# jdfxzzy/DPMN

Measured on AMD Instinct MI355X. Metric: SR images/sec (16x64->32x128, bs=48 per GPU, fp32 forward), higher is better.
Workload: dtype f32; 1 GPU; cfg1: TATT PSN + 3+3 PGRM (embed 96, windows 2/4/8) + CMM, forward-only; per_gpu_batch=48, global_batch=48, ranks=1, batches_in_flight=2, parallelism=dp1 (independent batch shards, no forward collective)

## Files before the change

dpmn_amd/_abi.py:

```python
import ctypes as C
import os

import torch

_HERE = os.path.dirname(os.path.abspath(__file__))
LIB_PATH = os.environ.get("DPMN_HIP_LIB") or os.path.join(_HERE, "lib", "libdpmn_hip.so")

if not os.path.exists(LIB_PATH):
    raise RuntimeError(
        "dpmn_amd: %s not found -- build it with `python -c 'import __graft_entry__ as g; g.build()'` "
        "(or `make -C dpmn_amd/csrc`).  There is no CPU fallback for the DPMN hot path." % LIB_PATH)

lib = C.CDLL(LIB_PATH)

fp = C.c_void_p


class PgrmBlock(C.Structure):
    _fields_ = [(n, fp) for n in (
        "norm1_q_w", "norm1_q_b", "norm1_kv_w", "norm1_kv_b", "q_w", "q_b", "kv_w", "kv_b")] + [
        ("bias_table", fp * 4)] + [(n, fp) for n in (
            "sk_proj_w", "sk_proj_b", "sk_fc1_w", "sk_fc1_b", "sk_fc2_w", "sk_fc2_b", "sk_head_w", "sk_head_b",
            "norm2_w", "norm2_b", "fc1_w", "fc1_b", "dw_w", "dw_b", "pw_w", "pw_b", "fc2_w", "fc2_b")]

# ... 114 lines not shown
    "dpmn_sk_mlp_in_supported": (_i, [_i, _i, _i, _i, _i]),
    "dpmn_pointwise_f32": (_i, [fp, fp, fp, fp, _i, _i, _i, fp]),
    "dpmn_conv2d_nhwc_f32": (_i, [C.POINTER(ConvDesc), fp]),
    "dpmn_distill_workspace_bytes": (_sz, [_i, _i, _i]),
    "dpmn_distill_forward_f32": (_i, [C.POINTER(DistillParams), fp, fp, _i, fp, fp, fp, fp, fp, _sz, _i, _i, _i, fp]),
    "dpmn_distill_backward_f32": (_i, [C.POINTER(DistillParams), C.POINTER(DistillGrads), fp, fp, fp, fp, fp, fp, fp, fp, fp, _sz, _i, _i, _i, fp]),
    "dpmn_conv2d_wgrad_unpack_multi_f32": (_i, [fp, fp, _i, _i, fp]),
    "dpmn_tl_interp_f32": (_i, [fp, fp, _i, _i, _i, _i, _i, fp]),
    "dpmn_pointwise_wgrad_det_bytes": (_sz, [_i, _i]),
    "dpmn_reduce_defer_begin": (_i, []),
    "dpmn_reduce_defer_enable": (_i, [_i]),
    "dpmn_reduce_defer_push": (_i, [C.POINTER(TnPending)]),
    "dpmn_reduce_defer_pending": (_i, []),
    "dpmn_reduce_defer_flush": (_i, [_i, fp]),
    "dpmn_xred_fallbacks": (_i, [C.POINTER(C.c_uint), _i]),
    "dpmn_selftest_xshfl": (_i, [C.POINTER(C.c_uint)]),
    "dpmn_selftest_lds_poison": (_i, [C.c_uint, _i, fp]),
    "dpmn_xred_test_force_recompute": (_i, [_i]),
    "dpmn_xred_enable": (_i, [_i]),
    "dpmn_nchw_to_nhwc_f32": (_i, [fp, fp, _i, _i, _i, _i, _i, fp]),
    "dpmn_nhwc_to_nchw_f32": (_i, [fp, fp, _i, _i, _i, _i, fp]),
    "dpmn_se_gate_f32": (_i, [fp, fp, fp, fp, fp, fp, fp, _i, _i, _i, _i, fp]),
    "dpmn_bigru_f32": (_i, [fp, fp, fp, fp, fp, _i, _i, _i, C.c_long, C.c_long, C.c_long, _i, fp]),
    "dpmn_small_linear_f32": (_i, [fp, fp, _i, fp, fp, fp, _i, _i, _i, _i, _f, fp]),
    "dpmn_tatt_encoder_layer_f32": (_i, [fp, fp, _PP, fp, _i, _i, _i, _i, fp]),
    "dpmn_cross_attn_f32": (_i, [fp, fp, fp, fp, fp, _i, _i, _i, _i, _i, fp]),
    "dpmn_add_layernorm64_f32": (_i, [fp, fp, fp, fp, fp, fp, fp, fp, _f, _i, C.c_long, fp]),
    "dpmn_cross_attn_qproj_f32": (_i, [fp, fp, fp, fp, fp, fp, fp, fp, _i, _i, _i, _i, _i, fp]),
    "dpmn_tatt_dec_tail_f32": (_i, [fp, fp, C.POINTER(TattDecLayer), fp, fp, fp, fp, _f, _i, C.c_long, fp]),
    "dpmn_gru_gate_f32": (_i, [fp, fp, fp, fp, C.c_long, _i, _i, fp]),
    "dpmn_to_mask_f32": (_i, [fp, C.c_long, fp, _i, _i, _i, fp]),
    "dpmn_mha32_f32": (_i, [fp, fp, _i, _i, _i, _f, fp]),
    "dpmn_layernorm_std_f32": (_i, [fp, fp, fp, _f, fp, _l, _i, fp]),
    "dpmn_rotate_img_f32": (_i, [fp, fp, fp, _f, fp, _i, _i, _i, _i, fp]),
    "dpmn_blend_f32": (_i, [fp, C.c_long, fp, C.c_long, fp, _f, _i, _i, fp]),
    "dpmn_psnr_ssim_workspace_bytes": (_sz, [_i, _i, _i, _i]),
    "dpmn_psnr_ssim_f32": (_i, [fp, C.c_long, fp, C.c_long, fp, fp, _i, _i, _i, _i, fp]),
    "dpmn_gemm_tn_f32": (_i, [fp, fp, fp, fp, _i, _i, _i, fp, _sz, fp]),
    "dpmn_gemm_tn_partial_bytes": (_sz, [_i, _i, _i]),
    "dpmn_gemm_tn_partial_f32": (_i, [fp, fp, fp, fp, _i, _i, _i, fp, _sz, C.POINTER(TnPending), fp]),
    "dpmn_tn_reduce_multi_f32": (_i, [C.POINTER(TnPending), _i, fp]),
    "dpmn_gemm_tn_group_f32": (_i, [C.POINTER(TnItem), _i, fp]),
    "dpmn_colsum_f32": (_i, [fp, fp, C.c_long, _i, fp]),
    "dpmn_colsum_det_f32": (_i, [fp, fp, C.c_long, _i, fp, _sz, fp]),
    "dpmn_layernorm_bwd_f32": (_i, [fp, fp, fp, _f, fp, _i, fp, fp, C.c_long, _i, fp]),
    "dpmn_layernorm_bwd_det_f32": (_i, [fp, fp, fp, _f, fp, _i, fp, fp, C.c_long, _i, fp, _sz, fp]),
# ... 259 lines not shown
```

dpmn_amd/csrc/common.h:

```cpp
#pragma once
#include <hip/hip_runtime.h>
#include <stdint.h>
#include <atomic>
#include "../../include/dpmn_hip.h"

typedef float f32x4 __attribute__((ext_vector_type(4)));

#define DPMN_CHECK_LAUNCH()                                                         \
  do {                                                                              \
    hipError_t e__ = hipGetLastError();                                             \
    if (e__ != hipSuccess) return dpmn_set_error(DPMN_ERR_LAUNCH, hipGetErrorString(e__)); \
  } while (0)

#define DPMN_REQUIRE(cond, msg)                                    \
  do {                                                             \
    if (!(cond)) return dpmn_set_error(DPMN_ERR_ARG, msg);         \
  } while (0)

int dpmn_set_error(int code, const char* msg);

__device__ __forceinline__ f32x4 mfma16(float a, float b, f32x4 c) {
  return __builtin_amdgcn_mfma_f32_16x16x4f32(a, b, c, 0, 0, 0);
}

// ... 123 lines not shown
__device__ __forceinline__ float drop_scale(unsigned long long seed, unsigned long long idx, float p, float inv_keep) {
  return drop_scale_z(drop_z0(seed, idx), p, inv_keep);
}

static inline hipStream_t as_stream(dpmn_stream_t s) { return (hipStream_t)s; }

constexpr int DPMN_MAX_DEVICES = 64;
int dpmn_cu_count();
int dpmn_lds_limit();
template <auto Kernel>
inline void dpmn_lds_optin(size_t bytes) {
  static std::atomic<int> set[DPMN_MAX_DEVICES];
  int dev = -1;
  const bool keyed = hipGetDevice(&dev) == hipSuccess && dev >= 0 && dev < DPMN_MAX_DEVICES;
  if (keyed && (int)bytes <= set[dev].load(std::memory_order_relaxed)) return;
  if (hipFuncSetAttribute(reinterpret_cast<const void*>(Kernel), hipFuncAttributeMaxDynamicSharedMemorySize, (int)bytes) == hipSuccess && keyed)
    set[dev].store((int)bytes, std::memory_order_relaxed);
}

enum ProfTag { PT_CONV_IGEMM_128 = 0, PT_CONV_IGEMM_64, PT_CONV_IGEMM_NARROW, PT_CONV_SPLITK_REDUCE, PT_CONV_HALO, PT_CONV_HALO_C4,
               PT_GEMM_PW, PT_GEMM_WSTAT, PT_GEMM_KLOOP, PT_DWCONV_GELU, PT_WATTN8, PT_WATTN_SCALAR, PT_ATTN_FUSED, PT_BIGRU,
               PT_MHA32, PT_PATCH_EMBED, PT_SK_GATE, PT_TAIL, PT_GEMM_WSTAT_LN, PT_CONV_IGEMM_SK, PT_ATTN_FUSED_BWD, PT_WATTN_BWD,
               PT_CONV_WGRAD, PT_GEMM_TN, PT_TN_REDUCE, PT_DWCONV_BWD, PT_WGRAD_UNPACK, PT_CONV_PACK, PT_AFFINE_ACT_BWD, PT_LN_BWD, PT_WATTN_MFMA32, PT_CROSS_ATTN,
               PT_TATT_DEC_TAIL, PT_COUNT };
extern unsigned long long g_dpmn_prof_mask;
extern double g_dpmn_prof_hint_bytes;
extern int g_dpmn_bf16;
extern int g_dpmn_x3;
typedef __bf16 bf16x2 __attribute__((ext_vector_type(2)));
typedef __bf16 bf16x8 __attribute__((ext_vector_type(8)));
__device__ __forceinline__ uint2 pack_bf16x4(float a, float b, float c, float d) {
  typedef float f32x2_ __attribute__((ext_vector_type(2)));
  const bf16x2 lo = __builtin_convertvector((f32x2_){a, b}, bf16x2), hi = __builtin_convertvector((f32x2_){c, d}, bf16x2);
  return make_uint2(__builtin_bit_cast(unsigned, lo), __builtin_bit_cast(unsigned, hi));
}
__device__ __forceinline__ f32x4 mfma16_bf16(bf16x8 a, bf16x8 b, f32x4 c) {
  return __builtin_amdgcn_mfma_f32_16x16x32_bf16(a, b, c, 0, 0, 0);
}
__device__ __forceinline__ void x3_split2t(float a, float b, unsigned& h, unsigned& m, unsigned& l) {
  const unsigned ua = __float_as_uint(a), ub = __float_as_uint(b);
  h = __builtin_amdgcn_perm(ub, ua, 0x07060302u);
  const float ra = a - __uint_as_float(ua & 0xffff0000u), rb = b - __uint_as_float(ub & 0xffff0000u);
  const unsigned va = __float_as_uint(ra), vb = __float_as_uint(rb);
  m = __builtin_amdgcn_perm(vb, va, 0x07060302u);
  const float sa = ra - __uint_as_float(va & 0xffff0000u), sb = rb - __uint_as_float(vb & 0xffff0000u);
  l = __builtin_amdgcn_perm(__float_as_uint(sb), __float_as_uint(sa), 0x07060302u);
}
// ... 24 lines not shown
```

dpmn_amd/csrc/psn_forward.hip:

```cpp
#include "common.h"

namespace {
struct PsnWs {
  float *r1, *r2, *gi, *s, *f[2], *t, *u;
  size_t total;
};
PsnWs carve(const dpmn_psn_weights* w, int B, int H, int W, char* base) {
  size_t off = 0;
  auto take = [&](size_t n) {
    float* p = base ? reinterpret_cast<float*>(base + off) : nullptr;
    off += ((n * sizeof(float) + 255) / 256) * 256;
    return p;
  };
  const size_t px = (size_t)B * H * W, ch = w->ch;
  PsnWs s;
  s.r1 = take(px * ch); s.r2 = take(px * ch); s.gi = take(px * 6 * w->hidden); s.s = take(px * ch);
  s.f[0] = take(px * ch); s.f[1] = take(px * ch); s.t = take(px * ch); s.u = take(px * 4 * ch);
  s.total = off;
  return s;
}
dpmn_conv_desc conv_same(const float* in, int cin, int B, int H, int W, int k, const float* wp, const float* bias, int cout, float* out,
                         const dpmn_cmm_scratch* sc) {
  dpmn_conv_desc d{};
  d.in[0] = in; d.cseg[0] = cin;
// ... 11 lines not shown
size_t dpmn_psn_trunk_workspace_bytes(const dpmn_psn_weights* w, int B, int H, int W) {
  if (!w || B <= 0 || H <= 0 || W <= 0) return 0;
  return carve(w, B, H, W, nullptr).total;
}

int dpmn_psn_trunk_f32(const dpmn_psn_weights* w, const float* b1, const float* tp, int tp_channels, float* out, void* workspace,
                       size_t workspace_bytes, const dpmn_cmm_scratch* sc, int B, int H, int W, dpmn_stream_t stream) {
  DPMN_REQUIRE(w && b1 && out && workspace && sc, "psn_trunk: null pointer");
  DPMN_REQUIRE(B >= 1 && w->srb_nums >= 1 && w->srb_nums <= 8 && w->ch == 2 * w->hidden, "psn_trunk: bad shape (1..8 SRBs, ch = 2 * hidden)");
  DPMN_REQUIRE((tp == nullptr) == (tp_channels == 0), "psn_trunk: tp and tp_channels go together");
  PsnWs s = carve(w, B, H, W, static_cast<char*>(workspace));
  if (s.total > workspace_bytes) return dpmn_set_error(DPMN_ERR_WORKSPACE, "psn_trunk: workspace too small");
  const int ch = w->ch, M = B * H * W, hid = w->hidden;
  int rc;
#define RUN(call) do { rc = (call); if (rc != DPMN_OK) return rc; } while (0)
  const float* f = b1;
  for (int i = 0; i < w->srb_nums; ++i) {
    const dpmn_psn_srb& p = w->srb[i];
    dpmn_conv_desc d1 = conv_same(f, ch, B, H, W, 3, p.c1_w, p.c1_b, ch, s.r1, sc);
    d1.epi_act = DPMN_ACT_MISH;
    RUN(dpmn_conv2d_nhwc_f32(&d1, stream));
    dpmn_conv_desc d2 = conv_same(s.r1, ch, B, H, W, 3, p.c2_w, p.c2_b, ch, s.r2, sc);
    RUN(dpmn_conv2d_nhwc_f32(&d2, stream));
    if (tp) RUN(dpmn_cat2_linear_f32(s.r2, ch, tp, tp_channels, p.g1_w, p.g1_b, s.gi, M, 6 * hid, DPMN_ACT_NONE, stream));
    else RUN(dpmn_linear_f32(s.r2, p.g1_w, p.g1_b, nullptr, nullptr, s.gi, M, 6 * hid, ch, DPMN_ACT_NONE, 0.f, stream));
    RUN(dpmn_bigru_f32(s.gi, p.g1_whh, p.g1_bhh, f, s.s, B * W, H, W, (long)H * W, 1, W, hid, stream));
    RUN(dpmn_linear_f32(s.s, p.g2_w, p.g2_b, nullptr, nullptr, s.gi, M, 6 * hid, ch, DPMN_ACT_NONE, 0.f, stream));
    float* fo = s.f[i & 1];
    RUN(dpmn_bigru_f32(s.gi, p.g2_whh, p.g2_bhh, nullptr, fo, B * H, W, 1, W, 0, 1, hid, stream));
    f = fo;
  }
  dpmn_conv_desc d7 = conv_same(f, ch, B, H, W, 3, w->b7_w, w->b7_b, ch, s.t, sc);
  d7.res = b1;
  RUN(dpmn_conv2d_nhwc_f32(&d7, stream));
  dpmn_conv_desc du = conv_same(s.t, ch, B, H, W, 3, w->up_w, w->up_b, 4 * ch, s.u, sc);
  du.epi_act = DPMN_ACT_MISH; du.pixel_shuffle = 1;
  RUN(dpmn_conv2d_nhwc_f32(&du, stream));
  dpmn_conv_desc dl = conv_same(s.u, ch, B, 2 * H, 2 * W, 9, w->last_w, w->last_b, w->in_planes, out, sc);
  dl.epi_act = DPMN_ACT_TANH; dl.out_nchw = 1;
  RUN(dpmn_conv2d_nhwc_f32(&dl, stream));
#undef RUN
  return DPMN_OK;
}

}

namespace {
struct TpiWs {
  float *src, *mem, *q, *k, *v, *o, *t1, *out[2], *f;
  size_t total;
};
TpiWs carve_tpi(int B, int L, int S, int E, char* base) {
// ... 69 lines not shown
```

dpmn_amd/csrc/runtime.hip:

```cpp
#include "common.h"
#include <string.h>
#include <stdlib.h>

static thread_local char g_err[512] = "";

int dpmn_set_error(int code, const char* msg) {
  strncpy(g_err, msg ? msg : "", sizeof(g_err) - 1);
  g_err[sizeof(g_err) - 1] = 0;
  return code;
}

int dpmn_cu_count() {
  static std::atomic<int> cus[DPMN_MAX_DEVICES];
  int dev = -1;
  if (hipGetDevice(&dev) != hipSuccess) return 256;
  const bool keyed = dev >= 0 && dev < DPMN_MAX_DEVICES;
  int n = keyed ? cus[dev].load(std::memory_order_relaxed) : 0;
  if (n < 1) {
    if (hipDeviceGetAttribute(&n, hipDeviceAttributeMultiprocessorCount, dev) != hipSuccess || n < 1) return 256;
    if (keyed) cus[dev].store(n, std::memory_order_relaxed);
  }
  return n;
}

int dpmn_lds_limit() {
  static std::atomic<int> lds[DPMN_MAX_DEVICES];
  int dev = -1;
  if (hipGetDevice(&dev) != hipSuccess) return 65536;
  const bool keyed = dev >= 0 && dev < DPMN_MAX_DEVICES;
  int n = keyed ? lds[dev].load(std::memory_order_relaxed) : 0;
  if (n < 1) {
    if (hipDeviceGetAttribute(&n, hipDeviceAttributeMaxSharedMemoryPerBlock, dev) != hipSuccess || n < 1) return 65536;
    if (keyed) lds[dev].store(n, std::memory_order_relaxed);
  }
  return n;
}

unsigned long long g_dpmn_prof_mask = 0ull;
double g_dpmn_prof_hint_bytes = 0.0;
int g_dpmn_x3 = 0;
int g_dpmn_bf16 = 0;
namespace {
const char* const kTagNames[PT_COUNT] = {
    "k_conv_igemm<128,128>", "k_conv_igemm<64,64>", "k_conv_igemm<128,16|32>", "k_conv_splitk_reduce", "k_conv_halo", "k_conv_halo_c4",
    "k_gemm_pw", "k_gemm_wstat|rowreg", "k_gemm_kloop", "k_dwconv_gelu", "k_window_attn8_mfma", "k_window_attn<2|4>", "k_ln_qkv_window_attn",
    "k_bigru", "k_mha32", "k_patch_embed_ln", "k_sk_gate", "k_tail_conv2", "k_gemm_wstat|rowreg<LN prologue>", "k_conv_igemm_sk", "k_ln_qkv_window_attn_bwd", "k_window_attn_bwd_mfma",
    "k_conv_wgrad", "k_gemm_tn_reg", "k_tn_reduce_multi", "k_dwconv_bwd", "k_wgrad_unpack_multi", "k_conv_pack_multi", "k_affine_act_bwd", "k_ln_bwd", "k_window_attn_mfma<4|8|16,32>", "k_cross_attn",
    "k_tatt_dec_tail"};
struct Rec { int tag; double flops, bytes; };
struct Prof {
  int cap = 0, count = 0, limit = 0;
  hipEvent_t* ev = nullptr;
  Rec* rec = nullptr;
} g_prof;
}

int dpmn_prof_open(int tag, hipStream_t st, double flops, double bytes) {
  if (g_prof.count >= g_prof.limit) return -1;
  const int i = g_prof.count++;
  g_prof.rec[i] = Rec{tag, flops, bytes};
  (void)hipEventRecord(g_prof.ev[2 * i], st);
  return i;
}
void dpmn_prof_close(int slot, hipStream_t st) { (void)hipEventRecord(g_prof.ev[2 * slot + 1], st); }

extern "C" {
int dpmn_abi_version(void) { return 5; }
int dpmn_set_compute_dtype(int mode) {
  DPMN_REQUIRE(mode >= 0 && mode <= 2, "set_compute_dtype: 0 = f32, 1 = bf16 operands, 2 = f32 via three bf16 terms");
  g_dpmn_bf16 = mode == 1;
  g_dpmn_x3 = mode == 2;
// ... 46 lines not shown
```

dpmn_amd/csrc/tatt.hip:

```cpp
#include "common.h"

namespace {

typedef float v2f __attribute__((ext_vector_type(2)));

template <int HID>
__global__ __launch_bounds__(256) void k_bigru(const float* gi, const float* w_hh ,
                                                const float* b_hh , const float* res,
                                                float* out, int nseq, int T, int inner, long outer_stride,
                                                long inner_stride, long step_stride) {
  static_assert(HID == 32, "lane mapping assumes 32 hidden units per direction");
  __shared__ __attribute__((aligned(16))) float hs[4][64];
  const int wave = threadIdx.x >> 6, lane = threadIdx.x & 63;
  const int dir = lane >> 5, j = lane & 31;
  const long s = (long)blockIdx.x * 4 + wave;
  if (s >= nseq) return;
  v2f wrz[HID], wnn[HID / 2];
  const float* wb = w_hh + (size_t)dir * 3 * HID * HID;
#pragma unroll
  for (int k = 0; k < HID; ++k) wrz[k] = v2f{wb[(size_t)j * HID + k], wb[(size_t)(HID + j) * HID + k]};
#pragma unroll
  for (int k = 0; k < HID / 2; ++k) wnn[k] = v2f{wb[(size_t)(2 * HID + j) * HID + 2 * k], wb[(size_t)(2 * HID + j) * HID + 2 * k + 1]};
  const float br = b_hh[dir * 3 * HID + j], bz = b_hh[dir * 3 * HID + HID + j], bn = b_hh[dir * 3 * HID + 2 * HID + j];
  asm volatile("" ::: "memory");
// ... 51 lines not shown
    h = (1.f - z) * n + z * h;
    op[0] = fmaf(g4[3], rmul, h);
    op += rd;
  };
  fetch(g0);
  fetch(g1);
  fetch(g2);
  int t = 0;
  for (; t + 3 < T; t += 4) {
    fetch(g3);
    step(g0, t);
    fetch(g0);
    step(g1, t + 1);
    fetch(g1);
    step(g2, t + 2);
    fetch(g2);
    step(g3, t + 3);
  }
  if (t < T) step(g0, t);
  if (t + 1 < T) step(g1, t + 1);
  if (t + 2 < T) step(g2, t + 2);
}

__global__ __launch_bounds__(256) void k_small_linear_tiled(const float* __restrict__ x, const float* __restrict__ add, int add_rows,
                                                             const float* __restrict__ w, const float* __restrict__ b,
                                                             float* __restrict__ y, int M, int N, int K, int act, float slope) {
  __shared__ float xs[32][64];
  __shared__ float ws[64][65];
  const int m0 = blockIdx.x * 32, n0 = blockIdx.y * 64;
  const int c = threadIdx.x & 63, r = threadIdx.x >> 6;
  float acc[8];
#pragma unroll
  for (int i = 0; i < 8; ++i) acc[i] = (b && n0 + c < N) ? b[n0 + c] : 0.f;
  for (int k0 = 0; k0 < K; k0 += 64) {
    const int kc = K - k0 < 64 ? K - k0 : 64;
    for (int e = threadIdx.x; e < 32 * 64; e += 256) {
      const int row = e >> 6, k = e & 63, m = m0 + row;
      float v = 0.f;
      if (m < M && k < kc) {
        v = x[(size_t)m * K + k0 + k];
        if (add) v = v + add[(size_t)(m % add_rows) * K + k0 + k];
      }
      xs[row][k] = v;
    }
    for (int e = threadIdx.x; e < 64 * 64; e += 256) {
      const int col = e >> 6, k = e & 63;
// ... 483 lines not shown
  const int c = (idx % c4) * 4;
  const int x = (idx / c4) % W, n = idx / ((long)c4 * W * H);
  const float sx = W > 1 ? (float)x * ((float)(Win - 1) / (float)(W - 1)) : 0.f;
  int x0 = (int)sx;
  if (x0 > Win - 1) x0 = Win - 1;
  const int x1 = x0 + 1 < Win ? x0 + 1 : Win - 1;
  const float l1 = sx - (float)x0, l0 = 1.f - l1;
  const float4 a = *reinterpret_cast<const float4*>(in + ((size_t)n * Win + x0) * C + c);
  const float4 b = *reinterpret_cast<const float4*>(in + ((size_t)n * Win + x1) * C + c);
  *reinterpret_cast<float4*>(out + idx * 4) = make_float4(l0 * a.x + l1 * b.x, l0 * a.y + l1 * b.y, l0 * a.z + l1 * b.z, l0 * a.w + l1 * b.w);
}

}

extern "C" {

int dpmn_bigru_f32(const float* gi, const float* w_hh, const float* b_hh, const float* res, float* out, int nseq, int T,
                   int inner, long outer_stride, long inner_stride, long step_stride, int hidden, dpmn_stream_t stream) {
  DPMN_REQUIRE(gi && w_hh && b_hh && out && nseq > 0 && T > 0 && inner > 0, "bigru: bad arguments");
  DPMN_REQUIRE(hidden == 32, "bigru: built for hidden_units=32 per direction (hd_u default, main.py:47)");
  ProfScope prof(PT_BIGRU, as_stream(stream), 2.0 * 2 * 3 * 32 * 32 * (double)nseq * T, 4.0 * (2 * 96 + 64 + 64) * (double)nseq * T);
  hipLaunchKernelGGL((k_bigru<32>), dim3((unsigned)((nseq + 3) / 4)), dim3(256), 0, as_stream(stream), gi, w_hh, b_hh, res, out,
                     nseq, T, inner, outer_stride, inner_stride, step_stride);
  DPMN_CHECK_LAUNCH();
  return DPMN_OK;
}

int dpmn_small_linear_f32(const float* x, const float* add, int add_rows, const float* w, const float* b, float* y, int M,
                          int N, int K, int act, float slope, dpmn_stream_t stream) {
  DPMN_REQUIRE(x && w && y && M > 0 && N > 0 && K > 0, "small_linear: bad arguments");
  hipLaunchKernelGGL(k_small_linear_tiled, dim3((unsigned)((M + 31) / 32), (unsigned)((N + 63) / 64)), dim3(256), 0, as_stream(stream), x,
                     add, add_rows > 0 ? add_rows : 1, w, b, y, M, N, K, act, slope);
  DPMN_CHECK_LAUNCH();
  return DPMN_OK;
}

int dpmn_tatt_encoder_layer_f32(const float* src, const float* pos, const float* const* w12, float* mem, int N, int L,
                                int E, int nhead, dpmn_stream_t stream) {
  DPMN_REQUIRE(src && pos && w12 && mem && N > 0, "encoder_layer: bad arguments");
  DPMN_REQUIRE(E == 64 && nhead == 4 && L <= 32, "encoder_layer: built for d_model=64, 4 heads, <=32 tokens (tatt.py:171-178)");
  EncW w{w12[0], w12[1], w12[2], w12[3], w12[4], w12[5], w12[6], w12[7], w12[8], w12[9], w12[10], w12[11]};
  hipLaunchKernelGGL((k_encoder_layer<64, 4>), dim3(N), dim3(256), 0, as_stream(stream), src, pos, w, mem, L);
  DPMN_CHECK_LAUNCH();
  return DPMN_OK;
}

// ... 81 lines not shown
```

dpmn_amd/model/tsrn.py:

```python
import math
import os

import torch
import torch.nn as nn

from .. import ops
from . import packing


NATIVE_TRUNK = os.environ.get("DPMN_PSN_NATIVE", "1") != "0"


class _GruBlock(nn.Module):
    def __init__(self, cin, cout):
        super().__init__()
        self.conv1 = nn.Conv2d(cin, cout, 1)
        self.gru = nn.GRU(cout, cout // 2, bidirectional=True, batch_first=True)


class _SRB(nn.Module):
    def __init__(self, ch, text_ch=0):
        super().__init__()
        self.conv1 = nn.Conv2d(ch, ch, 3, padding=1)
        self.bn1 = nn.BatchNorm2d(ch)
# ... 74 lines not shown
            P["up"] = packing.pack_conv(b8[0].conv.weight, b8[0].conv.bias)
            P["last"] = packing.pack_conv(b8[1].weight, b8[1].bias)
            self._extra_pack(P)
        self._pk = (key, P)
        return P

    def _extra_pack(self, P):
        pass

    def _pack_block_extra(self, P, i, blk):
        P["srb%d.g1" % i] = _pack_gru_block(blk.gru1)
        P["srb%d.g2" % i] = _pack_gru_block(blk.gru2)

    def _check_mode(self):
        if self.training:
            raise NotImplementedError("dpmn_amd PSN: only eval mode is built (DPMN keeps the PSN frozen in .eval(), "
                                      "super_resolution.py:56-59)")

    def _srb(self, x, P, i, tp=None):
        B, H, W, Cc = x.shape
        r = ops.conv2d([x], *P["srb%d.c1" % i], Cc, 3, pad=1, epi_act="mish")
        r = ops.conv2d([r], *P["srb%d.c2" % i], Cc, 3, pad=1)
        w1, b1, whh1, bhh1 = P["srb%d.g1" % i]
        M = B * H * W
        if tp is None:
            gi = ops.linear(r.reshape(M, Cc), w1, b1)
        else:
            gi = ops.cat2_linear(r.reshape(M, Cc), tp.reshape(M, tp.shape[3]), w1, b1)
        s = ops.bigru(gi, whh1, bhh1, B, H, W, "h", res=x)
        w2, b2, whh2, bhh2 = P["srb%d.g2" % i]
        gi = ops.linear(s.reshape(M, Cc), w2, b2)
        return ops.bigru(gi, whh2, bhh2, B, H, W, "w")

    def _native(self, P):
        from .. import _abi
        nat = getattr(self, "_nat", None)
        if nat is not None and nat[0] is P:
            return nat[1], nat[2]
        w = _abi.PsnWeights()
        w.in_planes, w.ch, w.hidden, w.srb_nums = self.in_planes, self.ch, self.ch // 2, self.srb_nums
        keep = []
        for i in range(self.srb_nums):
            q = w.srb[i]
            (q.c1_w, q.c1_b), (q.c2_w, q.c2_b) = [(t.data_ptr() for t in P["srb%d.c%d" % (i, j)]) for j in (1, 2)]
            for g in (1, 2):
                gw, gb, whh, bhh = P["srb%d.g%d" % (i, g)]
                setattr(q, "g%d_w" % g, gw.data_ptr()); setattr(q, "g%d_b" % g, gb.data_ptr())
                setattr(q, "g%d_whh" % g, whh.data_ptr()); setattr(q, "g%d_bhh" % g, bhh.data_ptr())
        (w.b7_w, w.b7_b), (w.up_w, w.up_b), (w.last_w, w.last_b) = [(t.data_ptr() for t in P[k]) for k in ("b7", "up", "last")]
        self._nat = (P, w, keep)
        if not hasattr(self, "_native_ws"):
            self._native_ws = {}
        return w, keep
# ... 95 lines not shown
```

dpmn_amd/ops.py:

```python
import torch
from ._abi import stream_of as _abi_stream_of

from . import _abi
from ._abi import dptr, lib, check, stream

ACT = {"none": 0, "gelu": 1, "relu": 2, "leaky02": 3, "leaky001": 4, "mish": 5, "prelu": 6, "tanh": 7, "sigmoid": 8,
       "relu_post_res": 9}


def linear(x, w, bias=None, res1=None, res2=None, act="none", slope=0.0):
    M, K = x.shape
    N = w.shape[0]
    y = torch.empty(M, N, device=x.device)
    check(lib.dpmn_linear_f32(dptr(x), dptr(w), dptr(bias, True), dptr(res1, True), dptr(res2, True), dptr(y), M, N, K,
                              ACT[act], float(slope), stream()))
    return y


def add_linear(x, addv, w, bias=None, act="none"):
    M, K = x.shape
    N = w.shape[0]
    y = torch.empty(M, N, device=x.device)
    check(lib.dpmn_add_linear_f32(dptr(x), dptr(addv), dptr(w), dptr(bias, True), dptr(y), M, N, K, ACT[act], stream()))
    return y
# ... 1373 lines not shown
    return out


def se_gate(x, fc1_w, fc1_b, fc2_w, fc2_b):
    B, H, W, Cc = x.shape
    out = torch.empty_like(x)
    hid = torch.empty(B, fc1_w.shape[0], device=x.device)
    check(lib.dpmn_se_gate_f32(dptr(x), dptr(fc1_w), dptr(fc1_b), dptr(fc2_w), dptr(fc2_b), dptr(out), dptr(hid), B, H * W,
                               Cc, fc1_w.shape[0], stream()))
    return out


def bigru(gi, w_hh, b_hh, B, H, W, axis, res=None, hidden=32):
    out = torch.empty(B, H, W, 2 * hidden, device=gi.device)
    if axis == "w":
        nseq, T, inner, outer, inner_s, step = B * H, W, 1, W, 0, 1
    else:
        nseq, T, inner, outer, inner_s, step = B * W, H, W, H * W, 1, W
    check(lib.dpmn_bigru_f32(dptr(gi), dptr(w_hh), dptr(b_hh), dptr(res, True), dptr(out), nseq, T, inner, outer, inner_s,
                             step, hidden, stream()))
    return out


def small_linear(x, w, b=None, add=None, act="none", slope=0.0):
    M, K = x.shape
    N = w.shape[0]
    y = torch.empty(M, N, device=x.device)
    check(lib.dpmn_small_linear_f32(dptr(x), dptr(add, True), 0 if add is None else add.shape[0], dptr(w), dptr(b, True),
                                    dptr(y), M, N, K, ACT[act], float(slope), stream()))
    return y


def tatt_encoder_layer(src, pos, w12, nhead=4):
    N, L, E = src.shape
    mem = torch.empty_like(src)
    check(lib.dpmn_tatt_encoder_layer_f32(dptr(src), dptr(pos), _abi.ptr_array(w12), dptr(mem), N, L, E, nhead, stream()))
    return mem


def cross_attn(q, k, v, nhead=4, need_weights=False):
    N, L, E = q.shape
    S = k.shape[1]
    o = torch.empty_like(q)
    pw = torch.empty(N, L, S, device=q.device) if need_weights else None
    check(lib.dpmn_cross_attn_f32(dptr(q), dptr(k), dptr(v), dptr(o), dptr(pw, True), N, L, S, E, nhead, stream()))
    return o, pw
# ... 677 lines not shown
```

include/dpmn_hip.h:

```cpp
#ifndef DPMN_HIP_H
#define DPMN_HIP_H

#include <stddef.h>
#include <stdint.h>

#ifdef __cplusplus
extern "C" {
#endif

typedef void* dpmn_stream_t;

enum { DPMN_OK = 0, DPMN_ERR_ARG = -1, DPMN_ERR_LAUNCH = -2, DPMN_ERR_WORKSPACE = -3, DPMN_ERR_RUNTIME = -4 };

enum { DPMN_ACT_NONE = 0, DPMN_ACT_GELU = 1, DPMN_ACT_RELU = 2, DPMN_ACT_LEAKY02 = 3, DPMN_ACT_LEAKY001 = 4,
       DPMN_ACT_MISH = 5, DPMN_ACT_PRELU = 6, DPMN_ACT_TANH = 7, DPMN_ACT_SIGMOID = 8,
       DPMN_ACT_RELU_POST_RES = 9  };

int dpmn_abi_version(void);
const char* dpmn_last_error(void);
int dpmn_set_compute_dtype(int mode);
int dpmn_get_compute_dtype(void);

int dpmn_linear_f32(const float* x, const float* w, const float* bias, const float* res1, const float* res2,
                    float* y, int M, int N, int K, int act, float slope, dpmn_stream_t stream);
// ... 107 lines not shown
  long long* bn1_nbt;
  const float *conv_feat_w, *conv_feat_b;
  const float *bn2_w, *bn2_b;
  float *bn2_rm, *bn2_rv;
  long long* bn2_nbt;
} dpmn_distill_params;
typedef struct {
  float *dconv_cat_w, *dconv_cat_b, *dbn1_w, *dbn1_b, *dconv_feat_w, *dconv_feat_b, *dbn2_w, *dbn2_b;
} dpmn_distill_grads;
size_t dpmn_distill_workspace_bytes(int B, int H, int W);
int dpmn_distill_forward_f32(const dpmn_distill_params* p, const float* x_deep, const float* x_shallow, int training, float* r,
                             float* state, float* feat, float* loss, void* workspace, size_t workspace_bytes, int B, int H, int W,
                             dpmn_stream_t stream);
int dpmn_distill_backward_f32(const dpmn_distill_params* p, const dpmn_distill_grads* g, const float* x_deep, const float* x_shallow,
                              const float* r, const float* state, const float* dfeat, const float* gloss, float* dx_deep,
                              float* dx_shallow, void* workspace, size_t workspace_bytes, int B, int H, int W, dpmn_stream_t stream);

int dpmn_se_gate_f32(const float* x, const float* fc1_w, const float* fc1_b, const float* fc2_w, const float* fc2_b,
                     float* out, float* hidden_ws, int B, int P, int C, int Cmid, dpmn_stream_t stream);

int dpmn_bigru_f32(const float* gi, const float* w_hh, const float* b_hh, const float* res, float* out, int nseq,
                   int T, int inner, long outer_stride, long inner_stride, long step_stride, int hidden,
                   dpmn_stream_t stream);
int dpmn_small_linear_f32(const float* x, const float* add, int add_rows, const float* w, const float* b, float* y,
                          int M, int N, int K, int act, float slope, dpmn_stream_t stream);
int dpmn_tatt_encoder_layer_f32(const float* src, const float* pos, const float* const* w12, float* mem, int N,
                                int L, int E, int nhead, dpmn_stream_t stream);
int dpmn_cross_attn_f32(const float* q, const float* k, const float* v, float* o, float* pw, int N, int L, int S, int E,
                        int nhead, dpmn_stream_t stream);
int dpmn_tl_interp_f32(const float* in, float* out, int N, int Win, int C, int H, int W, dpmn_stream_t stream);
int dpmn_add_layernorm64_f32(const float* x, const float* res, const float* g, const float* b, float* y,
                             const float* g2, const float* b2, float* acc_out, float alpha, int accumulate, long M,
                             dpmn_stream_t stream);
int dpmn_gru_gate_f32(const float* gi, const float* gh, float* h, float* hist, long hist_row_stride, int R, int H,
                      dpmn_stream_t stream);

int dpmn_patch_embed_ln_f32(const float* img, int cin, const float* pf_w, const float* pf_b, const float* pe_w,
                            const float* pe_b, const float* ln_w, const float* ln_b, float* tokens, int B, int Hi,
                            int Wi, int patch, int C, dpmn_stream_t stream);
int dpmn_patch_embed_ln_drop_f32(const float* img, int cin, const float* pf_w, const float* pf_b, const float* pe_w,
                                 const float* pe_b, const float* ln_w, const float* ln_b, float* tokens, int B, int Hi, int Wi,
                                 int patch, int C, float p_drop, unsigned long long seed, dpmn_stream_t stream);
int dpmn_window_attn_f32(const float* q, const float* kv, const float* const* bias_tables, const int* windows,
                         const int* shifts, int n_groups, int heads_per_group, float* out, int B, int H, int W,
                         int C, dpmn_stream_t stream);
int dpmn_sk_gate_f32(const float* colsum_partials, int parts_per_image, int L, const float* fc1_w,
// ... 456 lines not shown
```

Before: 6562 images/s.

## Fuse GRU input projection into bidirectional GRU recurrence kernel

Adds a k_bigru_proj kernel that computes the 6*hid input-gate projection with MFMA from LDS-resident weights per 16-step chunk, then runs the recurrence in the same wave. Both the C++ PSN path and the Python TSRN block use it when the shape is supported. This removes the gi intermediate buffer's global write and read and one launch per GRU. The cost is extra LDS, per-chunk prefetch logic, and a grid capped at the CU count, which may limit occupancy for the serial recurrence.

```diff
diff --git a/dpmn_amd/_abi.py b/dpmn_amd/_abi.py
--- a/dpmn_amd/_abi.py
+++ b/dpmn_amd/_abi.py
@@ -160,6 +160,8 @@
     "dpmn_nhwc_to_nchw_f32": (_i, [fp, fp, _i, _i, _i, _i, fp]),
     "dpmn_se_gate_f32": (_i, [fp, fp, fp, fp, fp, fp, fp, _i, _i, _i, _i, fp]),
     "dpmn_bigru_f32": (_i, [fp, fp, fp, fp, fp, _i, _i, _i, C.c_long, C.c_long, C.c_long, _i, fp]),
+    "dpmn_bigru_proj_supported": (_i, [_i, _i, _i]),
+    "dpmn_bigru_proj_f32": (_i, [fp, _i, fp, _i, fp, fp, fp, fp, fp, fp, _i, _i, _i, C.c_long, C.c_long, C.c_long, _i, fp]),
     "dpmn_small_linear_f32": (_i, [fp, fp, _i, fp, fp, fp, _i, _i, _i, _i, _f, fp]),
     "dpmn_tatt_encoder_layer_f32": (_i, [fp, fp, _PP, fp, _i, _i, _i, _i, fp]),
     "dpmn_cross_attn_f32": (_i, [fp, fp, fp, fp, fp, _i, _i, _i, _i, _i, fp]),
diff --git a/dpmn_amd/csrc/common.h b/dpmn_amd/csrc/common.h
--- a/dpmn_amd/csrc/common.h
+++ b/dpmn_amd/csrc/common.h
@@ -169,7 +169,7 @@
                PT_GEMM_PW, PT_GEMM_WSTAT, PT_GEMM_KLOOP, PT_DWCONV_GELU, PT_WATTN8, PT_WATTN_SCALAR, PT_ATTN_FUSED, PT_BIGRU,
                PT_MHA32, PT_PATCH_EMBED, PT_SK_GATE, PT_TAIL, PT_GEMM_WSTAT_LN, PT_CONV_IGEMM_SK, PT_ATTN_FUSED_BWD, PT_WATTN_BWD,
                PT_CONV_WGRAD, PT_GEMM_TN, PT_TN_REDUCE, PT_DWCONV_BWD, PT_WGRAD_UNPACK, PT_CONV_PACK, PT_AFFINE_ACT_BWD, PT_LN_BWD, PT_WATTN_MFMA32, PT_CROSS_ATTN,
-               PT_TATT_DEC_TAIL, PT_COUNT };
+               PT_TATT_DEC_TAIL, PT_BIGRU_PROJ, PT_COUNT };
 extern unsigned long long g_dpmn_prof_mask;
 extern double g_dpmn_prof_hint_bytes;
 extern int g_dpmn_bf16;
diff --git a/dpmn_amd/csrc/psn_forward.hip b/dpmn_amd/csrc/psn_forward.hip
--- a/dpmn_amd/csrc/psn_forward.hip
+++ b/dpmn_amd/csrc/psn_forward.hip
@@ -57,12 +57,22 @@
     RUN(dpmn_conv2d_nhwc_f32(&d1, stream));
     dpmn_conv_desc d2 = conv_same(s.r1, ch, B, H, W, 3, p.c2_w, p.c2_b, ch, s.r2, sc);
     RUN(dpmn_conv2d_nhwc_f32(&d2, stream));
-    if (tp) RUN(dpmn_cat2_linear_f32(s.r2, ch, tp, tp_channels, p.g1_w, p.g1_b, s.gi, M, 6 * hid, DPMN_ACT_NONE, stream));
-    else RUN(dpmn_linear_f32(s.r2, p.g1_w, p.g1_b, nullptr, nullptr, s.gi, M, 6 * hid, ch, DPMN_ACT_NONE, 0.f, stream));
-    RUN(dpmn_bigru_f32(s.gi, p.g1_whh, p.g1_bhh, f, s.s, B * W, H, W, (long)H * W, 1, W, hid, stream));
-    RUN(dpmn_linear_f32(s.s, p.g2_w, p.g2_b, nullptr, nullptr, s.gi, M, 6 * hid, ch, DPMN_ACT_NONE, 0.f, stream));
+    const bool fuse1 = dpmn_bigru_proj_supported(hid, ch, tp ? tp_channels : 0), fuse2 = dpmn_bigru_proj_supported(hid, ch, 0);
+    if (fuse1) {
+      RUN(dpmn_bigru_proj_f32(s.r2, ch, tp, tp ? tp_channels : 0, p.g1_w, p.g1_b, p.g1_whh, p.g1_bhh, f, s.s, B * W, H, W, (long)H * W, 1, W,
+                              hid, stream));
+    } else {
+      if (tp) RUN(dpmn_cat2_linear_f32(s.r2, ch, tp, tp_channels, p.g1_w, p.g1_b, s.gi, M, 6 * hid, DPMN_ACT_NONE, stream));
+      else RUN(dpmn_linear_f32(s.r2, p.g1_w, p.g1_b, nullptr, nullptr, s.gi, M, 6 * hid, ch, DPMN_ACT_NONE, 0.f, stream));
+      RUN(dpmn_bigru_f32(s.gi, p.g1_whh, p.g1_bhh, f, s.s, B * W, H, W, (long)H * W, 1, W, hid, stream));
+    }
     float* fo = s.f[i & 1];
-    RUN(dpmn_bigru_f32(s.gi, p.g2_whh, p.g2_bhh, nullptr, fo, B * H, W, 1, W, 0, 1, hid, stream));
+    if (fuse2) {
+      RUN(dpmn_bigru_proj_f32(s.s, ch, nullptr, 0, p.g2_w, p.g2_b, p.g2_whh, p.g2_bhh, nullptr, fo, B * H, W, 1, W, 0, 1, hid, stream));
+    } else {
+      RUN(dpmn_linear_f32(s.s, p.g2_w, p.g2_b, nullptr, nullptr, s.gi, M, 6 * hid, ch, DPMN_ACT_NONE, 0.f, stream));
+      RUN(dpmn_bigru_f32(s.gi, p.g2_whh, p.g2_bhh, nullptr, fo, B * H, W, 1, W, 0, 1, hid, stream));
+    }
     f = fo;
   }
   dpmn_conv_desc d7 = conv_same(f, ch, B, H, W, 3, w->b7_w, w->b7_b, ch, s.t, sc);
diff --git a/dpmn_amd/csrc/runtime.hip b/dpmn_amd/csrc/runtime.hip
--- a/dpmn_amd/csrc/runtime.hip
+++ b/dpmn_amd/csrc/runtime.hip
@@ -46,7 +46,7 @@
     "k_gemm_pw", "k_gemm_wstat|rowreg", "k_gemm_kloop", "k_dwconv_gelu", "k_window_attn8_mfma", "k_window_attn<2|4>", "k_ln_qkv_window_attn",
     "k_bigru", "k_mha32", "k_patch_embed_ln", "k_sk_gate", "k_tail_conv2", "k_gemm_wstat|rowreg<LN prologue>", "k_conv_igemm_sk", "k_ln_qkv_window_attn_bwd", "k_window_attn_bwd_mfma",
     "k_conv_wgrad", "k_gemm_tn_reg", "k_tn_reduce_multi", "k_dwconv_bwd", "k_wgrad_unpack_multi", "k_conv_pack_multi", "k_affine_act_bwd", "k_ln_bwd", "k_window_attn_mfma<4|8|16,32>", "k_cross_attn",
-    "k_tatt_dec_tail"};
+    "k_tatt_dec_tail", "k_bigru_proj"};
 struct Rec { int tag; double flops, bytes; };
 struct Prof {
   int cap = 0, count = 0, limit = 0;
diff --git a/dpmn_amd/csrc/tatt.hip b/dpmn_amd/csrc/tatt.hip
--- a/dpmn_amd/csrc/tatt.hip
+++ b/dpmn_amd/csrc/tatt.hip
@@ -97,6 +97,153 @@
   if (t + 2 < T) step(g2, t + 2);
 }
 
+typedef float f32x4_ __attribute__((ext_vector_type(4)));
+constexpr int BGP_WAVES = 4;
+constexpr int BGP_SLAB = 100;
+constexpr size_t bgp_lds_bytes(int cin) { return sizeof(float) * ((size_t)192 * (cin + 4) + 192 + BGP_WAVES * (2 * 16 * BGP_SLAB + 64)); }
+
+template <int CIN, bool RES>
+__global__ __launch_bounds__(BGP_WAVES * 64) void k_bigru_proj(const float* x, int c1, const float* x2, const float* w_ih ,
+                                                                const float* b_ih, const float* w_hh ,
+                                                                const float* b_hh , const float* res, float* out,
+                                                                int nseq, int T, int inner, long outer_stride, long inner_stride,
+                                                                long step_stride) {
+  constexpr int HID = 32, NQ = CIN / 16, WS = CIN + 4;
+  extern __shared__ __attribute__((aligned(16))) float bgp_smem[];
+  float* ws = bgp_smem;
+  float* bs = ws + 192 * WS;
+  const int wave = threadIdx.x >> 6, lane = threadIdx.x & 63;
+  float* slab = bs + 192 + wave * (2 * 16 * BGP_SLAB);
+  float* hs = bs + 192 + BGP_WAVES * (2 * 16 * BGP_SLAB) + wave * 64;
+  const int dir = lane >> 5, j = lane & 31;
+  const int c2 = CIN - c1;
+  v2f wrz[HID], wnn[HID / 2];
+  const float* wb = w_hh + (size_t)dir * 3 * HID * HID;
+#pragma unroll
+  for (int k = 0; k < HID; ++k) wrz[k] = v2f{wb[(size_t)j * HID + k], wb[(size_t)(HID + j) * HID + k]};
+#pragma unroll
+  for (int k = 0; k < HID / 2; ++k) wnn[k] = v2f{wb[(size_t)(2 * HID + j) * HID + 2 * k], wb[(size_t)(2 * HID + j) * HID + 2 * k + 1]};
+  const float br = b_hh[dir * 3 * HID + j], bz = b_hh[dir * 3 * HID + HID + j], bn = b_hh[dir * 3 * HID + 2 * HID + j];
+  for (int i = threadIdx.x; i < 192 * (CIN / 4); i += BGP_WAVES * 64) {
+    const int n = i / (CIN / 4), k4 = i % (CIN / 4);
+    *reinterpret_cast<float4*>(ws + n * WS + 4 * k4) = *reinterpret_cast<const float4*>(w_ih + (size_t)n * CIN + 4 * k4);
+  }
+  if (threadIdx.x < 192) bs[threadIdx.x] = b_ih[threadIdx.x];
+  __syncthreads();
+
+  const int ar = lane & 15, ag = lane >> 4;
+  auto pkfma = [](v2f a, v2f b, v2f c) -> v2f { return v2f{fmaf(a.x, b.x, c.x), fmaf(a.y, b.y, c.y)}; };
+  const int nch = (T + 15) >> 4;
+  float4 af[NQ], ab[NQ];
+  float rv[16];
+  auto seq_base = [&](long s) { return (s / inner) * outer_stride + (s % inner) * inner_stride; };
+  auto load_chunk = [&](long base, int c) {
+    const int tc = min(16 * c + ar, T - 1);
+    const long pf = base + (long)tc * step_stride, pb = base + (long)(T - 1 - tc) * step_stride;
+#pragma unroll
+    for (int q = 0; q < NQ; ++q) {
+      const int k = 16 * q + 4 * ag;
+      const bool first = 16 * q < c1;
+      const float* rf = first ? x + pf * c1 + k : x2 + pf * c2 + (k - c1);
+      const float* rb = first ? x + pb * c1 + k : x2 + pb * c2 + (k - c1);
+      af[q] = *reinterpret_cast<const float4*>(rf);
+      ab[q] = *reinterpret_cast<const float4*>(rb);
+    }
+    if constexpr (RES) {
+#pragma unroll
+      for (int tt = 0; tt < 16; ++tt) {
+        const int t = min(16 * c + tt, T - 1);
+        rv[tt] = res[(base + (long)(dir ? T - 1 - t : t) * step_stride) * (2 * HID) + dir * HID + j];
+      }
+    }
+    asm volatile("" ::: "memory");
+  };
+  const long s0 = (long)blockIdx.x * BGP_WAVES + wave, sstep = (long)gridDim.x * BGP_WAVES;
+  if (s0 < nseq) load_chunk(seq_base(s0), 0);
+  for (long s = s0; s < nseq; s += sstep) {
+    const long base = seq_base(s);
+    float h = 0.f;
+    float* op = out + (base + (dir ? (long)(T - 1) * step_stride : 0)) * (2 * HID) + dir * HID + j;
+    const long od = (dir ? -step_stride : step_stride) * (2 * HID);
+    for (int c = 0; c < nch; ++c) {
+#pragma unroll
+      for (int d = 0; d < 2; ++d) {
+#pragma unroll
+        for (int tg = 0; tg < 2; ++tg) {
+          f32x4_ acc[3];
+          const float* wp[3];
+#pragma unroll
+          for (int i = 0; i < 3; ++i) {
+            const int n = d * 96 + (tg * 3 + i) * 16 + ar;
+            const float b = bs[n];
+            acc[i] = f32x4_{b, b, b, b};
+            wp[i] = ws + n * WS + 4 * ag;
+          }
+#pragma unroll
+          for (int q = 0; q < NQ; ++q) {
+            const float4 a = d ? ab[q] : af[q];
+#pragma unroll
+            for (int i = 0; i < 3; ++i) {
+              const float4 b = *reinterpret_cast<const float4*>(wp[i] + 16 * q);
+              acc[i] = __builtin_amdgcn_mfma_f32_16x16x4f32(a.x, b.x, acc[i], 0, 0, 0);
+              acc[i] = __builtin_amdgcn_mfma_f32_16x16x4f32(a.y, b.y, acc[i], 0, 0, 0);
+              acc[i] = __builtin_amdgcn_mfma_f32_16x16x4f32(a.z, b.z, acc[i], 0, 0, 0);
+              acc[i] = __builtin_amdgcn_mfma_f32_16x16x4f32(a.w, b.w, acc[i], 0, 0, 0);
+            }
+          }
+#pragma unroll
+          for (int i = 0; i < 3; ++i)
+#pragma unroll
+            for (int e = 0; e < 4; ++e) slab[(d * 16 + 4 * ag + e) * BGP_SLAB + (tg * 3 + i) * 16 + ar] = acc[i][e];
+        }
+      }
+      float rc[16];
+#pragma unroll
+      for (int tt = 0; tt < 16; ++tt) rc[tt] = RES ? rv[tt] : 0.f;
+      const bool more = c + 1 < nch;
+      load_chunk(more ? base : seq_base(s + sstep < nseq ? s + sstep : s), more ? c + 1 : 0);
+      __builtin_amdgcn_wave_barrier();
+      const int nst = min(16, T - 16 * c);
+      const float* gp = slab + dir * 16 * BGP_SLAB + j;
+#pragma unroll
+      for (int tt = 0; tt < 16; ++tt) {
+        if (tt < nst) {
+          const float gr = gp[tt * BGP_SLAB], gz = gp[tt * BGP_SLAB + HID], gn = gp[tt * BGP_SLAB + 2 * HID];
+          hs[lane] = h;
+          __builtin_amdgcn_wave_barrier();
+          v2f rz0 = {br, bz}, rz1 = {0.f, 0.f}, n0 = {bn, 0.f}, n1 = {0.f, 0.f};
+          const float* hp = hs + dir * HID;
+#pragma unroll
+          for (int k = 0; k < HID; k += 8) {
+            const float4 h0 = *reinterpret_cast<const float4*>(hp + k);
+            const float4 h1 = *reinterpret_cast<const float4*>(hp + k + 4);
+            rz0 = pkfma(wrz[k], v2f{h0.x, h0.x}, rz0);
+            rz1 = pkfma(wrz[k + 1], v2f{h0.y, h0.y}, rz1);
+            n0 = pkfma(wnn[k / 2], v2f{h0.x, h0.y}, n0);
+            rz0 = pkfma(wrz[k + 2], v2f{h0.z, h0.z}, rz0);
+            rz1 = pkfma(wrz[k + 3], v2f{h0.w, h0.w}, rz1);
+            n1 = pkfma(wnn[k / 2 + 1], v2f{h0.z, h0.w}, n1);
+            rz0 = pkfma(wrz[k + 4], v2f{h1.x, h1.x}, rz0);
+            rz1 = pkfma(wrz[k + 5], v2f{h1.y, h1.y}, rz1);
+            n0 = pkfma(wnn[k / 2 + 2], v2f{h1.x, h1.y}, n0);
+            rz0 = pkfma(wrz[k + 6], v2f{h1.z, h1.z}, rz0);
+            rz1 = pkfma(wrz[k + 7], v2f{h1.w, h1.w}, rz1);
+            n1 = pkfma(wnn[k / 2 + 3], v2f{h1.z, h1.w}, n1);
+          }
+          __builtin_amdgcn_wave_barrier();
+          const float r = sigmoid_fast(gr + (rz0.x + rz1.x));
+          const float z = sigmoid_fast(gz + (rz0.y + rz1.y));
+          const float n = tanh_fast(gn + r * ((n0.x + n1.x) + (n0.y + n1.y)));
+          h = (1.f - z) * n + z * h;
+          op[0] = RES ? rc[tt] + h : h;
+          op += od;
+        }
+      }
+      __builtin_amdgcn_wave_barrier();
+    }
+  }
+}
+
 __global__ __launch_bounds__(256) void k_small_linear_tiled(const float* __restrict__ x, const float* __restrict__ add, int add_rows,
                                                              const float* __restrict__ w, const float* __restrict__ b,
                                                              float* __restrict__ y, int M, int N, int K, int act, float slope) {
@@ -626,6 +773,36 @@
   ProfScope prof(PT_BIGRU, as_stream(stream), 2.0 * 2 * 3 * 32 * 32 * (double)nseq * T, 4.0 * (2 * 96 + 64 + 64) * (double)nseq * T);
   hipLaunchKernelGGL((k_bigru<32>), dim3((unsigned)((nseq + 3) / 4)), dim3(256), 0, as_stream(stream), gi, w_hh, b_hh, res, out,
                      nseq, T, inner, outer_stride, inner_stride, step_stride);
+  DPMN_CHECK_LAUNCH();
+  return DPMN_OK;
+}
+
+int dpmn_bigru_proj_supported(int hidden, int c1, int c2) {
+  return hidden == 32 && c1 > 0 && c2 >= 0 && c1 % 16 == 0 && c2 % 16 == 0 && (c1 + c2 == 64 || c1 + c2 == 128);
+}
+
+int dpmn_bigru_proj_f32(const float* x, int c1, const float* x2, int c2, const float* w_ih, const float* b_ih, const float* w_hh,
+                        const float* b_hh, const float* res, float* out, int nseq, int T, int inner, long outer_stride,
+                        long inner_stride, long step_stride, int hidden, dpmn_stream_t stream) {
+  DPMN_REQUIRE(x && w_ih && b_ih && w_hh && b_hh && out && nseq > 0 && T > 0 && inner > 0, "bigru_proj: bad arguments");
+  DPMN_REQUIRE((x2 != nullptr) == (c2 > 0), "bigru_proj: x2 and c2 go together");
+  DPMN_REQUIRE(dpmn_bigru_proj_supported(hidden, c1, c2), "bigru_proj: built for hidden 32 and c1 + c2 of 64 or 128 in multiples of 16");
+  const int cin = c1 + c2;
+  const double px = (double)nseq * T;
+  ProfScope prof(PT_BIGRU_PROJ, as_stream(stream), 2.0 * px * cin * 192 + 2.0 * px * 2 * 3 * 32 * 32,
+                 4.0 * (px * (cin + 64 + (res ? 64 : 0)) + 192.0 * (cin + 1) + 2 * 96 * 33));
+  const size_t lds = bgp_lds_bytes(cin);
+  const dim3 grid((unsigned)std::min((nseq + BGP_WAVES - 1) / BGP_WAVES, dpmn_cu_count())), block(BGP_WAVES * 64);
+  if (!x2) x2 = x;
+#define BGP_LAUNCH(CIN, RES)                                                                                                         \
+  do {                                                                                                                               \
+    dpmn_lds_optin<k_bigru_proj<CIN, RES>>(lds);                                                                                     \
+    hipLaunchKernelGGL((k_bigru_proj<CIN, RES>), grid, block, lds, as_stream(stream), x, c1, x2, w_ih, b_ih, w_hh, b_hh, res, out,   \
+                       nseq, T, inner, outer_stride, inner_stride, step_stride);                                                    \
+  } while (0)
+  if (cin == 64) { if (res) BGP_LAUNCH(64, true); else BGP_LAUNCH(64, false); }
+  else { if (res) BGP_LAUNCH(128, true); else BGP_LAUNCH(128, false); }
+#undef BGP_LAUNCH
   DPMN_CHECK_LAUNCH();
   return DPMN_OK;
 }
diff --git a/dpmn_amd/model/tsrn.py b/dpmn_amd/model/tsrn.py
--- a/dpmn_amd/model/tsrn.py
+++ b/dpmn_amd/model/tsrn.py
@@ -120,13 +120,16 @@
         r = ops.conv2d([x], *P["srb%d.c1" % i], Cc, 3, pad=1, epi_act="mish")
         r = ops.conv2d([r], *P["srb%d.c2" % i], Cc, 3, pad=1)
         w1, b1, whh1, bhh1 = P["srb%d.g1" % i]
-        M = B * H * W
-        if tp is None:
-            gi = ops.linear(r.reshape(M, Cc), w1, b1)
+        M, hid = B * H * W, Cc // 2
+        r, t2 = r.reshape(M, Cc), None if tp is None else tp.reshape(M, tp.shape[3])
+        if ops.bigru_proj_supported(hid, Cc, 0 if t2 is None else t2.shape[1]):
+            s = ops.bigru_proj(r, t2, w1, b1, whh1, bhh1, B, H, W, "h", res=x, hidden=hid)
         else:
-            gi = ops.cat2_linear(r.reshape(M, Cc), tp.reshape(M, tp.shape[3]), w1, b1)
-        s = ops.bigru(gi, whh1, bhh1, B, H, W, "h", res=x)
+            gi = ops.linear(r, w1, b1) if t2 is None else ops.cat2_linear(r, t2, w1, b1)
+            s = ops.bigru(gi, whh1, bhh1, B, H, W, "h", res=x)
         w2, b2, whh2, bhh2 = P["srb%d.g2" % i]
+        if ops.bigru_proj_supported(hid, Cc, 0):
+            return ops.bigru_proj(s.reshape(M, Cc), None, w2, b2, whh2, bhh2, B, H, W, "w", hidden=hid)
         gi = ops.linear(s.reshape(M, Cc), w2, b2)
         return ops.bigru(gi, whh2, bhh2, B, H, W, "w")
 
diff --git a/dpmn_amd/ops.py b/dpmn_amd/ops.py
--- a/dpmn_amd/ops.py
+++ b/dpmn_amd/ops.py
@@ -1419,6 +1419,22 @@
     return out
 
 
+def bigru_proj_supported(hidden, c1, c2=0):
+    return bool(lib.dpmn_bigru_proj_supported(int(hidden), int(c1), int(c2)))
+
+
+def bigru_proj(x, x2, w_ih, b_ih, w_hh, b_hh, B, H, W, axis, res=None, hidden=32):
+    out = torch.empty(B, H, W, 2 * hidden, device=x.device)
+    if axis == "w":
+        nseq, T, inner, outer, inner_s, step = B * H, W, 1, W, 0, 1
+    else:
+        nseq, T, inner, outer, inner_s, step = B * W, H, W, H * W, 1, W
+    check(lib.dpmn_bigru_proj_f32(dptr(x), x.shape[1], dptr(x2, True), 0 if x2 is None else x2.shape[1], dptr(w_ih), dptr(b_ih),
+                                  dptr(w_hh), dptr(b_hh), dptr(res, True), dptr(out), nseq, T, inner, outer, inner_s, step, hidden,
+                                  stream()))
+    return out
+
+
 def small_linear(x, w, b=None, add=None, act="none", slope=0.0):
     M, K = x.shape
     N = w.shape[0]
diff --git a/include/dpmn_hip.h b/include/dpmn_hip.h
--- a/include/dpmn_hip.h
+++ b/include/dpmn_hip.h
@@ -153,6 +153,10 @@
 int dpmn_bigru_f32(const float* gi, const float* w_hh, const float* b_hh, const float* res, float* out, int nseq,
                    int T, int inner, long outer_stride, long inner_stride, long step_stride, int hidden,
                    dpmn_stream_t stream);
+int dpmn_bigru_proj_supported(int hidden, int c1, int c2);
+int dpmn_bigru_proj_f32(const float* x, int c1, const float* x2, int c2, const float* w_ih, const float* b_ih, const float* w_hh,
+                        const float* b_hh, const float* res, float* out, int nseq, int T, int inner, long outer_stride,
+                        long inner_stride, long step_stride, int hidden, dpmn_stream_t stream);
 int dpmn_small_linear_f32(const float* x, const float* add, int add_rows, const float* w, const float* b, float* y,
                           int M, int N, int K, int act, float slope, dpmn_stream_t stream);
 int dpmn_tatt_encoder_layer_f32(const float* src, const float* pos, const float* const* w12, float* mem, int N,
```

Measured after the change: 6568 images/s, median of 4. No clear change (+0.1%).
